# agent-charon/MinGraph-UNet

Hardware: AMD Instinct MI355X
Metric: segmented Mpix/sec, full MinGraph-UNet forward (U-Net + patch-graph GAT), 512x512 batch (higher is better)
Workload: dtype f32

## Files before the change

include/mgunet.h:

```cpp
#ifndef MGUNET_H
#define MGUNET_H

#include <stddef.h>
#include <stdint.h>

#ifdef __cplusplus
extern "C" {
#endif

#define MGU_OK 0
#define MGU_ERR_INVALID -1
#define MGU_ERR_HIP -2
#define MGU_ERR_STATE -3
#define MGU_ERR_NOMEM -4

#define MGU_DTYPE_F32 0
#define MGU_DTYPE_BF16 1

typedef struct mgu_ctx mgu_ctx;

typedef struct {
  const char* name;
  const void* ptr;
  int64_t numel;
// ... 294 lines not shown
                            const float* shift_dev, int act, float* y_dev, int ldy, void* hip_stream);
int mgu_channel_sum_nhwc(mgu_ctx* ctx, const float* x_dev, int ldx, int64_t M, int C, float* out_dev, void* hip_stream);

int mgu_channel_sum_images_nhwc(mgu_ctx* ctx, const float* x_dev, int ldx, int B, int64_t M, int C, float* out_dev, void* hip_stream);

double mgu_unet_flops(mgu_ctx* ctx, int B, int H, int W);
double mgu_unet_mfma_flops(mgu_ctx* ctx, int B, int H, int W);
int mgu_profile_enable(mgu_ctx* ctx, int on);
typedef struct {
  const char* name;
  double ms, flops_alg, flops_mfma;
  int launches, pipe;
} mgu_kernel_stat;
int mgu_profile_read_kernels(mgu_ctx* ctx, mgu_kernel_stat* out, int cap, int* n_out);
int mgu_profile_read(mgu_ctx* ctx, double* conv_ms, int* conv_launches, double* total_ms);

#ifdef __cplusplus
}
#endif
#endif
```

mingraph-unet_amd/csrc/asm/lint_wino_asm.py:

```python
#!/usr/bin/env python3
import re
import sys


def regs(tok):
    tok = tok.strip().lstrip("-").strip("|")
    m = re.match(r"v\[(\d+):(\d+)\]$", tok)
    if m:
        return set(range(int(m.group(1)), int(m.group(2)) + 1))
    m = re.match(r"v(\d+)$", tok)
    return {int(m.group(1))} if m else set()


def parse(line):
    line = line.split(";")[0].strip()
    if not line or line.endswith(":") or line.startswith("."):
        return None
    parts = line.split(None, 1)
    op = parts[0]
    args = []
    if len(parts) > 1:
        a = re.split(r",\s*", parts[1])
        args = [x.split()[0] if x.split() else x for x in a]
    return op, args, line
# ... 50 lines not shown

def loop_bodies(lines):
    lab = {}
    for i, ln in enumerate(lines):
        m = re.match(r"^(\.\w+):", ln)
        if m:
            lab[m.group(1)] = i
    bodies = []
    for i, ln in enumerate(lines):
        m = re.match(r"\s*s_cbranch_scc1\s+(\.\w+)", ln)
        if m and m.group(1) in lab and lab[m.group(1)] < i:
            bodies.append((m.group(1), lines[lab[m.group(1)]:i]))
    return bodies


def replay(stream, errors, where, prime=()):
    vm, lg = [], []
    valu_age = {}
    mfma_age = {}
    prev = None
    m0_fresh = False
    held = {}
    writes = {}

    def age(n):
        for d in (valu_age, mfma_age):
            for r in list(d):
                d[r] += n
                if d[r] > 40:
                    del d[r]

# ... 44 lines not shown
                    errors.append(f"{where}: `{text}` reads v{r} {valu_age[r]} wait state(s) after a VALU write (2 required)")
        else:
            for r in touched if kind in ("valu", "lds_store", "lds_store_addtid", "vm_store", "readlane") else src:
                if r in src and mfma_age.get(r, 99) < 18:
                    errors.append(f"{where}: `{text}` reads MFMA result v{r} after {mfma_age[r]} wait states (18 required)")
        if op.endswith("_dpp"):
            for r in src:
                if valu_age.get(r, 99) < 2:
                    errors.append(f"{where}: `{text}` (DPP) reads v{r} {valu_age[r]} wait state(s) after a VALU write (2 required)")
        if kind == "valu" and prev and prev[0] in ("lds_store", "vm_store") and len(prev[1]) >= 4 and (dst & prev[1]):
            errors.append(f"{where}: `{text}` overwrites store data of the previous instruction `{prev[2]}`")
        if kind == "lds_store_addtid" and m0_fresh:
            errors.append(f"{where}: `{text}` directly behind the write of M0")
        if kind == "readlane" and any(valu_age.get(r, 99) < 1 for r in src):
            errors.append(f"{where}: `{text}` directly behind the VALU write of its source")
        if op in ("v_add_f32_e32", "v_sub_f32_e32"):
            hs = [held.get(r) for a in args[1:3] for r in sorted(regs(a))]
            if len(hs) == 2 and any(h and h[0] == "sum" for h in hs):
                if hs[0] and hs[1] and hs[0] != hs[1]:
                    o = hs[1] if hs[0][0] == "sum" else hs[0]
                    why = f"holds what `{o[1]}` wrote" if o[0] == "other" else \
                          "holds an LDS read, not an inner sum" if o[0] == "lds" else "holds an inner sum of another read base"
                    errors.append(f"{where}: `{text}` combines an inner sum with a register that {why}")
        age(1)
        if kind == "valu":
            for r in dst:
                valu_age[r] = 0
                mfma_age.pop(r, None)
        if kind == "mfma":
            for r in dst:
                mfma_age[r] = 0
# ... 14 lines not shown
        if kind == "vm_load":
            vm.append((dst, text))
        elif kind == "vm_store":
            vm.append((set(), text))
        elif kind == "lds_load":
            lg.append((dst, text))
        elif kind in ("lds_store", "lds_store_addtid"):
            lg.append((set(), text))
        m0_fresh = op == "s_mov_b32" and args and args[0] == "m0"
        data = set()
        if kind in ("lds_store", "vm_store"):
            data = regs(args[1]) if kind == "lds_store" else regs(args[0])
        prev = (kind, data, text)


def check(text):
    errors = []
    ks = kernels(text)
    for name, lines in ks.items():
        replay(lines, errors, f"{name} (straight line)")
        for lab, body in loop_bodies(lines):
            replay(body * 3, errors, f"{name} loop {lab}")
    return errors, len(ks)


if __name__ == "__main__":
    errs, n = check(open(sys.argv[1]).read())
    for e in errs[:40]:
        print(e)
    print(f"{n} kernels, {len(errs)} finding(s)")
    sys.exit(1 if errs else 0)
```

mingraph-unet_amd/csrc/common.h:

```cpp
#pragma once
#include <hip/hip_runtime.h>
#include <stdint.h>

#include "device.h"

namespace mgu {

inline int grid_for(int64_t work, int threads, int cap) {
  int64_t b = (work + threads - 1) / threads;
  if (b < 1) b = 1;
  if (b > cap) b = cap;
  return (int)b;
}
inline bool aligned16(const void* p) { return ((uintptr_t)p & 15) == 0; }

struct Tuning {
  bool first_mfma = true;
  bool use_wino = true;
  int wino_prec = 1;
  bool convt_frag = true;
  bool wino_cp = true;
  int wino_ppb_cap = 32;
  bool wgrad_halo = true;
  bool wino_wgrad = true;
  bool convt_dgrad_x3 = true;
  bool wgrad_x3 = true;
  bool wgrad_thin = true;
  bool wino_dgrad = true;
  bool gat_fused = true;
  bool head_fused = true;
  bool wino_asm = true;
  int fwd_groups = 2;
  int lovasz_passes = 4;
};
const Tuning& default_tuning();
hipError_t ensure_dyn_lds(const void* func, size_t bytes, bool (&done)[64]);

struct IgemmDesc {
  const Tuning* tn;
  const float* in;
  const float* w;
  const float* wu;
  const float* scale;
  const float* shift;
  float* out;
  int M;
// ... 28 lines not shown
};
inline size_t wino_head_psum_bytes(int B, int H, int W) { return (size_t)B * (H / 16) * (W / 16) * 8 * 32 * sizeof(float); }

inline const Tuning& tun(const IgemmDesc& d) { return d.tn ? *d.tn : default_tuning(); }
enum class ConvKernel {
  None,
  WinoAsmWide, WinoAsmCp1r2, WinoAsmCp1r4,
  WinoAsmCp1r2Head,
  WinoCp2, WinoCp1, WinoCp2Stats, WinoCp1Stats,
  WinoCp1Head,
  WinoF32Wide, WinoF32Narrow,
  WinoX3Wide, WinoX3Narrow,
  HaloF32, HaloBf16Np8, HaloBf16Np4,
  TilesF32, TilesBf16,
  ConvtX3, ConvtBf16f, ConvtX3Dgrad,
};
ConvKernel pick_conv(const IgemmDesc& d, int dtype, const WinoHead* head = nullptr);
hipError_t launch_conv(const IgemmDesc& d, ConvKernel k, int dtype, hipStream_t s, const WinoHead* head = nullptr);
inline bool conv_fuses_head(ConvKernel k) { return k == ConvKernel::WinoAsmCp1r2Head || k == ConvKernel::WinoCp1Head; }
inline hipError_t launch_igemm_f32(const IgemmDesc& d, hipStream_t s) { return launch_conv(d, pick_conv(d, 0), 0, s); }
inline hipError_t launch_igemm_bf16(const IgemmDesc& d, hipStream_t s) { return launch_conv(d, pick_conv(d, 1), 1, s); }
const char* conv_kernel_name(ConvKernel k, const IgemmDesc& d);
const char* conv_dgrad_name(ConvKernel k, const IgemmDesc& d);
struct ConvCost {
  double mfma;
  int pipe;
};
ConvCost conv_cost(ConvKernel k, const IgemmDesc& d);
inline bool conv_is_wino(ConvKernel k) { return k >= ConvKernel::WinoAsmWide && k <= ConvKernel::WinoX3Narrow; }
inline bool conv_fuses_pool(ConvKernel k) {
  return conv_is_wino(k) || (k >= ConvKernel::HaloF32 && k <= ConvKernel::HaloBf16Np4);
}
inline bool conv_reads_panel(ConvKernel k) {
  return !conv_is_wino(k) && k != ConvKernel::ConvtX3 && k != ConvKernel::ConvtBf16f && k != ConvKernel::ConvtX3Dgrad;
}
bool wino_layer(const Tuning& t, int KS, int Cp);
bool wino_dgrad_layer(const Tuning& t, int KS, int Cop);
bool convt_x3_layer(const Tuning& t, int Cin, int Cout);
bool convt_x3_dgrad_layer(const Tuning& t, int Cin, int Cout);
bool convt_bf16f_layer(const Tuning& t, int Cin, int Cout);
bool wino_head_layer(const Tuning& t, int dtype, int Cin, int ncls, int patch, int B, int H, int W);
inline bool wino_wide(const IgemmDesc& d) { return d.N > 32; }
struct WinoPlan {
  int tiles_x, tiles_y, total, nblk, ppb, ngroups, per_xcd;
};
WinoPlan wino_plan(const IgemmDesc& d);
int wino_grid_blocks(const IgemmDesc& d);
hipError_t launch_convt_x3(const IgemmDesc& d, hipStream_t s);
hipError_t launch_convt_bf16f(const IgemmDesc& d, hipStream_t s);
hipError_t launch_convt_x3_dgrad(const IgemmDesc& d, hipStream_t s);
bool first_mfma_applicable(int dtype, int Cin, int Cp, int Cout, int ldout, int coff, int64_t H, int64_t W);
hipError_t launch_first_mfma(int dtype, const void* in, const float* wfm, const float* scale, const float* shift, void* out, int B, int H,
                             int W, int ldout, int coff, int relu, hipStream_t s);
hipError_t launch_first_mfma_direct(int dtype, const float* x, int64_t sn, int64_t sc, int64_t sh, int64_t sw, int cin, const float* wfm,
                                    const float* scale, const float* shift, void* out, int B, int H, int W, int ldout, int coff, int relu,
                                    hipStream_t s);
bool first_conv_applicable(int dtype, int Cin, int Cp, int Cout, int ldout, int coff);
hipError_t launch_first_conv(int dtype, const void* in, const float* wf, const float* scale, const float* shift, void* out, int B, int H, int W,
                             int Cin, int Cout, int ldout, int coff, int relu, hipStream_t s);
hipError_t launch_wino_f32(const IgemmDesc& d, ConvKernel k, hipStream_t s, const WinoHead* head = nullptr);
hipError_t launch_patch_sum_combine(const float* psum, float* out, int nodes, hipStream_t s);
hipError_t launch_wino_cp_asm(const IgemmDesc& d, ConvKernel k, hipStream_t s, const WinoHead* head = nullptr);

// ... 136 lines not shown
```

mingraph-unet_amd/csrc/convt_x3.hip:

```cpp
#include <hip/hip_runtime.h>
#include <stdint.h>

#include <algorithm>
#include <type_traits>

#include "common.h"

namespace mgu {


namespace {

template <int MODE, int NI>
__global__ __launch_bounds__(256, 2) void convt2x2_x3_kernel(const float* __restrict__ in, const int ldin, const uint16_t* __restrict__ Wx,
                                                             const float* __restrict__ shift, float* __restrict__ out, const int M,
                                                             const int H, const int W, const int Cin, const int Cout, const int ldout,
                                                             const int coff, const int Hout, const int Wout, const int ntn,
                                                             const int nblocks) {
  constexpr int AP = 40, ABUF = 3 * 128 * AP;
  __shared__ __attribute__((aligned(16))) uint16_t As[2 * ABUF];
  __shared__ int rowoff[128];
  const int chunk = gridDim.x >> 3;
  const int lb = (blockIdx.x & 7) * chunk + (blockIdx.x >> 3);
  if (lb >= nblocks) return;
// ... 169 lines not shown

hipError_t launch_convt_x3_dgrad(const IgemmDesc& d, hipStream_t s) {
  const bool wide = (d.N & 127) == 0;
  const int mtiles = (d.M + 127) / 128, ntn = d.N / (wide ? 128 : 64);
  const int nb = mtiles * ntn;
  const int chunk = (nb + 7) / 8;
  if (wide)
    hipLaunchKernelGGL((convt2x2_x3_kernel<1, 2>), dim3(chunk * 8), dim3(256), 0, s, d.in, d.ldin, reinterpret_cast<const uint16_t*>(d.wu),
                       (const float*)nullptr, d.out, d.M, d.H, d.W, d.Cp, d.N, d.ldout, d.coff, d.Hout, d.Wout, ntn, nb);
  else
    hipLaunchKernelGGL((convt2x2_x3_kernel<1, 1>), dim3(chunk * 8), dim3(256), 0, s, d.in, d.ldin, reinterpret_cast<const uint16_t*>(d.wu),
                       (const float*)nullptr, d.out, d.M, d.H, d.W, d.Cp, d.N, d.ldout, d.coff, d.Hout, d.Wout, ntn, nb);
  return hipGetLastError();
}

hipError_t launch_convt_x3(const IgemmDesc& d, hipStream_t s) {
  const int mtiles = (d.M + 127) / 128, ntn = d.N / 128;
  const int nb = mtiles * ntn;
  const int chunk = (nb + 7) / 8;
  hipLaunchKernelGGL((convt2x2_x3_kernel<0, 2>), dim3(chunk * 8), dim3(256), 0, s, d.in, d.ldin, reinterpret_cast<const uint16_t*>(d.wu), d.shift, d.out,
                     d.M, d.H, d.W, d.Cp, d.ct_cout, d.ldout, d.coff, d.Hout, d.Wout, ntn, nb);
  return hipGetLastError();
}

}
```

mingraph-unet_amd/csrc/ctx.h:

```cpp
#pragma once
#include <stdarg.h>
#include <stdio.h>
#include <stdlib.h>
#include <string.h>

#include <map>
#include <string>
#include <vector>

#include "../../include/mgunet.h"
#include "common.h"

struct Layer {
  std::string prefix;
  std::string conv;
  std::string bn;
  int Cin = 0, Cp = 0, Cout = 0, KS = 3;
  bool convt = false;
  int K = 0, Kp = 0, N = 0, Np = 0;
  float *wp = nullptr, *scale = nullptr, *shift = nullptr;
  bool first = false;
  bool ctb = false;
  bool ctx3 = false;
  bool wino = false;
// ... 82 lines not shown
  hipStream_t comm_stream = nullptr;
  hipEvent_t comm_ev[16] = {};
  int comm_ev_next = 0;
  bool prof = false;
  std::vector<hipEvent_t> ev;
  struct ProfRec {
    const char* name;
    double alg, mfma;
    int pipe;
  };
  std::vector<ProfRec> prec;
  int ev_used = 0;
  hipEvent_t ev_total[2] = {nullptr, nullptr};
  hipStream_t fwd_stream = nullptr;
  hipEvent_t fwd_ev[2] = {nullptr, nullptr};
  int panel_packs = 0;
};

namespace mgud {

inline int rup(int v, int m) { return (v + m - 1) / m * m; }
extern std::string g_create_err;

inline Layer make_layer(int dtype, int Cin, int Cp, int Cout, int KS, bool convt) {
  Layer L;
  L.Cin = Cin, L.Cp = Cp, L.Cout = Cout, L.KS = KS, L.convt = convt;
  L.K = KS * KS * Cp, L.Kp = rup(L.K, dtype == MGU_DTYPE_BF16 ? 64 : 32);
  L.N = convt ? 4 * Cout : Cout, L.Np = rup(L.N, 128);
  return L;
}
// ... 208 lines not shown
```

mingraph-unet_amd/csrc/igemm.hip:

```cpp
#include "common.h"
#include <algorithm>
#include <type_traits>

namespace mgu {


const Tuning& default_tuning() {
  static const Tuning t;
  return t;
}

hipError_t ensure_dyn_lds(const void* func, size_t bytes, bool (&done)[64]) {
  if (bytes <= 65536) return hipSuccess;
  int dev = 0;
  hipError_t e = hipGetDevice(&dev);
  if (e != hipSuccess) return e;
  if (dev < 0 || dev >= 64) return hipFuncSetAttribute(func, hipFuncAttributeMaxDynamicSharedMemorySize, (int)bytes);
  if (done[dev]) return hipSuccess;
  e = hipFuncSetAttribute(func, hipFuncAttributeMaxDynamicSharedMemorySize, (int)bytes);
  if (e == hipSuccess) done[dev] = true;
  return e;
}

template <typename T> struct Elem;
// ... 651 lines not shown

static bool convt_x3_dgrad_applicable(const IgemmDesc& d) {
  return convt_x3_dgrad_layer(tun(d), d.N, d.Cp) && d.KS == 2 && d.wu && d.K == 4 * d.Cp && (d.ldin & 3) == 0 && !d.scale && !d.shift &&
         !d.relu && !d.split_n && !d.pool && (long)d.M * d.ldout < (1l << 31) && (long)d.Hout * d.Wout * d.ldin < (1l << 31);
}

ConvKernel pick_conv(const IgemmDesc& d, int dtype, const WinoHead* head) {
  using K = ConvKernel;
  if (d.M <= 0 || d.N <= 0) return K::None;
  if (dtype == 1) {
    if (d.out_mode == 1) return d.KS != 1 ? K::None : convt_bf16f_applicable(d) ? K::ConvtBf16f : K::TilesBf16;
    const int np = halo_np<__bf16>(d);
    if (np) return np == 8 ? K::HaloBf16Np8 : K::HaloBf16Np4;
    return d.KS == 3 || d.KS == 1 ? K::TilesBf16 : K::None;
  }
  if (d.out_mode == 1) return d.KS != 1 ? K::None : convt_x3_applicable(d) ? K::ConvtX3 : K::TilesF32;
  if (convt_x3_dgrad_applicable(d)) return K::ConvtX3Dgrad;
  if (wino_applicable(d)) {
    const Tuning& t = tun(d);
    const bool wide = wino_wide(d);
    if (!t.wino_prec) return wide ? K::WinoF32Wide : K::WinoF32Narrow;
    if (!t.wino_cp || (long)d.H * d.W * d.ldin * 4 >= 0x7fff0000l) return wide ? K::WinoX3Wide : K::WinoX3Narrow;
    if (d.stat_slots) return wide ? K::WinoCp2Stats : K::WinoCp1Stats;
    if (head && wino_head_applicable(d, *head)) return t.wino_asm ? K::WinoAsmCp1r2Head : K::WinoCp1Head;
    if (wino_asm_applicable(d)) return wide ? K::WinoAsmWide : d.Cp == 32 ? K::WinoAsmCp1r2 : K::WinoAsmCp1r4;
    return wide ? K::WinoCp2 : K::WinoCp1;
  }
  if (halo_np<float>(d) == 8) return K::HaloF32;
  return d.KS >= 1 && d.KS <= 3 ? K::TilesF32 : K::None;
}

// ... 1 lines not shown
  switch (k) {
    case ConvKernel::WinoAsmWide: return "mgu_wino_cp2_gfx950 (asm form of wino3x3_cp_kernel<2>)";
    case ConvKernel::WinoAsmCp1r2: return "mgu_wino_cp1r2_gfx950 (asm form of wino3x3_cp_kernel<1>)";
    case ConvKernel::WinoAsmCp1r4: return "mgu_wino_cp1r4_gfx950 (asm form of wino3x3_cp_kernel<1>)";
    case ConvKernel::WinoAsmCp1r2Head: return "mgu_wino_cp1r2h_gfx950 (asm form of wino3x3_cp_kernel<1, head>: + 1x1 head + patch sums)";
    case ConvKernel::WinoCp1Head: return "wino3x3_cp_kernel<1, head> (+ 1x1 head + patch sums)";
    case ConvKernel::WinoCp2: case ConvKernel::WinoCp2Stats: return "wino3x3_cp_kernel<2>";
    case ConvKernel::WinoCp1: case ConvKernel::WinoCp1Stats: return "wino3x3_cp_kernel<1>";
    case ConvKernel::WinoF32Wide: return "wino3x3_f32_kernel<0,0>";
    case ConvKernel::WinoF32Narrow: return "wino3x3_f32_kernel<1,0>";
    case ConvKernel::WinoX3Wide: return "wino3x3_f32_kernel<0,1>";
    case ConvKernel::WinoX3Narrow: return "wino3x3_f32_kernel<1,1>";
    case ConvKernel::HaloF32: return "conv3x3_halo_kernel<f32>";
    case ConvKernel::HaloBf16Np8: case ConvKernel::HaloBf16Np4: return "conv3x3_halo_kernel<bf16>";
    case ConvKernel::TilesBf16: return d.out_mode == 1 ? "igemm_kernel<bf16> (ConvTranspose)" : "igemm_kernel<bf16>";
    case ConvKernel::ConvtX3: return "convt2x2_x3_kernel";
    case ConvKernel::ConvtBf16f: return "convt2x2_bf16_kernel";
    case ConvKernel::ConvtX3Dgrad: return "convt2x2_x3_kernel<dgrad>";
    case ConvKernel::TilesF32: case ConvKernel::None: break;
  }
  return d.out_mode == 1 ? "igemm_kernel<f32> (ConvTranspose)" : d.KS == 2 ? "igemm_kernel<f32> (ConvTranspose dgrad)" : "igemm_kernel<f32>";
}

const char* conv_dgrad_name(ConvKernel k, const IgemmDesc& d) {
  switch (k) {
    case ConvKernel::WinoAsmWide: case ConvKernel::WinoCp2: case ConvKernel::WinoCp2Stats: return "wino3x3_cp_kernel<2> (dgrad)";
    case ConvKernel::WinoAsmCp1r2: case ConvKernel::WinoAsmCp1r4: case ConvKernel::WinoCp1: case ConvKernel::WinoCp1Stats:
    case ConvKernel::WinoAsmCp1r2Head: case ConvKernel::WinoCp1Head:
      return "wino3x3_cp_kernel<1> (dgrad)";
    case ConvKernel::WinoX3Wide: case ConvKernel::WinoX3Narrow: return "wino3x3_f32_kernel<*,1> (dgrad)";
    case ConvKernel::WinoF32Wide: case ConvKernel::WinoF32Narrow: return "wino3x3_f32_kernel<*,0> (dgrad)";
    case ConvKernel::ConvtX3Dgrad: return "convt2x2_x3_kernel (dgrad)";
    default: return d.KS == 2 ? "igemm_kernel<f32> (ConvTranspose dgrad)" : "igemm/halo (dgrad)";
  }
}

ConvCost conv_cost(ConvKernel k, const IgemmDesc& d) {
  const double direct = 2.0 * d.M * (double)d.K * d.N;
  switch (k) {
    case ConvKernel::WinoF32Wide: case ConvKernel::WinoF32Narrow:
      return {2.0 * (d.M / (d.H * d.W)) * ((d.H + 1) / 2) * ((d.W + 1) / 2) * 16.0 * d.Cp * d.N, 0};
    case ConvKernel::ConvtX3: case ConvKernel::ConvtX3Dgrad: return {6.0 * direct, 1};
    case ConvKernel::HaloBf16Np8: case ConvKernel::HaloBf16Np4: case ConvKernel::TilesBf16: case ConvKernel::ConvtBf16f: return {direct, 1};
    case ConvKernel::HaloF32: case ConvKernel::TilesF32: case ConvKernel::None: return {direct, 0};
    default:
      return {2.0 * (d.M / (d.H * d.W)) * ((d.H + 1) / 2) * ((d.W + 1) / 2) * 16.0 * d.Cp * d.N * 6.0, 1};
  }
}

hipError_t launch_conv(const IgemmDesc& d, ConvKernel k, int dtype, hipStream_t s, const WinoHead* head) {
  if (d.M <= 0 || d.N <= 0) return hipSuccess;
  if (dtype == 1) {
    if ((d.Cp & 7) || (d.ldin & 7) || (d.Kp % 64) || d.K > d.Kp || d.split_n) return hipErrorInvalidValue;
  } else {
    if ((d.Cp & 3) || (d.ldin & 3) || (d.Kp % 32) || d.K > d.Kp) return hipErrorInvalidValue;
  }
  if (conv_fuses_head(k) != (head != nullptr)) return hipErrorInvalidValue;
// ... 5 lines not shown
    case ConvKernel::WinoF32Wide: case ConvKernel::WinoF32Narrow: case ConvKernel::WinoX3Wide: case ConvKernel::WinoX3Narrow:
      return launch_wino_f32(d, k, s);
    case ConvKernel::HaloF32: return launch_halo_tiles<float, 8>(d, s);
    case ConvKernel::HaloBf16Np8: return launch_halo_tiles<__bf16, 8>(d, s);
    case ConvKernel::HaloBf16Np4: return launch_halo_tiles<__bf16, 4>(d, s);
    case ConvKernel::TilesF32:
      if (d.out_mode == 1) return launch_tiles<float, 1, 1>(d, s);
      if (d.KS == 3) return launch_tiles<float, 3, 0>(d, s);
      if (d.KS == 1) return launch_tiles<float, 1, 0>(d, s);
      return launch_tiles<float, 2, 0>(d, s);
    case ConvKernel::TilesBf16:
      if (d.out_mode == 1) return launch_tiles<__bf16, 1, 1>(d, s);
      if (d.KS == 3) return launch_tiles<__bf16, 3, 0>(d, s);
      return launch_tiles<__bf16, 1, 0>(d, s);
    case ConvKernel::ConvtX3: return launch_convt_x3(d, s);
    case ConvKernel::ConvtBf16f: return launch_convt_bf16f(d, s);
    case ConvKernel::ConvtX3Dgrad: return launch_convt_x3_dgrad(d, s);
    case ConvKernel::None: break;
  }
  return hipErrorInvalidValue;
}

}
```

mingraph-unet_amd/csrc/mgunet_api.hip:

```cpp
#include "ctx.h"

#include <algorithm>

using namespace mgu;
using namespace mgud;

namespace mgud {
std::string g_create_err;
}

namespace {

struct WsPlan {
  size_t xin, tmp, tmp_slice, bott, total;
  std::vector<size_t> pooled;
};

int fwd_groups(const mgu_ctx* c, int B) { return c->tn.fwd_groups >= 2 && B >= 2 ? 2 : 1; }
int group_images(const mgu_ctx* c, int B) { return (B + fwd_groups(c, B) - 1) / fwd_groups(c, B); }

WsPlan plan_ws(const mgu_ctx* c, int B, int H, int W) {
  std::vector<int> hs, wsz;
  level_dims(H, W, c->depth, hs, wsz);
  auto out = [&](const Block& b, int l) { return (size_t)B * hs[l] * wsz[l] * c->layers[b.conv2].Cout; };
// ... 62 lines not shown
  Tuning& t = c->tn;
  t.first_mfma = !flag("MGU_NO_FIRST_MFMA");
  t.use_wino = !flag("MGU_NO_WINOGRAD");
  t.wino_prec = num("MGU_WINO_PREC", t.wino_prec) ? 1 : 0;
  t.wino_cp = !flag("MGU_NO_WINO_CP");
  t.convt_frag = !flag("MGU_NO_CONVT_FRAG");
  t.wino_ppb_cap = std::max(1, num("MGU_WINO_PPB_CAP", 32));
  t.wgrad_halo = !flag("MGU_NO_WGRAD_HALO");
  t.wino_wgrad = !flag("MGU_NO_WINO_WGRAD");
  t.wgrad_x3 = !flag("MGU_NO_WGRAD_X3");
  t.convt_dgrad_x3 = !flag("MGU_NO_CONVT_DGRAD_X3");
  t.wgrad_thin = !flag("MGU_NO_THIN_WGRAD");
  t.wino_dgrad = !flag("MGU_NO_WINO_DGRAD");
  t.gat_fused = !flag("MGU_NO_GAT_FUSED");
  t.wino_asm = num("MGU_WINO_ASM", 1) > 0;
  t.head_fused = num("MGU_HEAD_FUSED", 1) > 0;
  t.fwd_groups = num("MGU_FWD_GROUPS", t.fwd_groups) >= 2 ? 2 : 1;
  t.lovasz_passes = num("MGU_LOVASZ_PASSES", t.lovasz_passes) == 3 ? 3 : 4;
  *out = c;
  return MGU_OK;
}

void mgu_destroy(mgu_ctx* c) {
  if (!c) return;
  (void)hipSetDevice(c->device);
  (void)hipDeviceSynchronize();
  (void)mgu_comm_destroy(c);
  if (c->arena) (void)hipFree(c->arena);
  if (c->ws) (void)hipFree(c->ws);
  if (c->gws) (void)hipFree(c->gws);
// ... 285 lines not shown
  if (d.stat_slots || d.pool) k = pick_conv(d, c->dtype, f.head);
  t.head = conv_fuses_head(k);
  const WinoHead* head = t.head ? f.head : nullptr;
  if (took) *took = t;
  if (L.wp_dirty && conv_reads_panel(k)) {
    HIPCHK(c, launch_pack_one(L.convt ? pack_convt_panel(L.w_src, L.wp, c->dtype, L.Cin, L.Cout, L.Kp)
                                      : pack_conv_panel(L.w_src, L.wp, c->dtype, L.Cout, L.Cin, L.Cp, L.KS, L.Kp), s));
    L.wp_dirty = false;
    ++c->panel_packs;
  }
  double alg = L.convt ? 2.0 * d.M * (double)L.Cin * L.Cout * 4.0 : 2.0 * d.M * (double)L.KS * L.KS * L.Cin * L.Cout;
  if (head) alg += 2.0 * d.M * (double)L.Cout * head->ncls;
  const ConvCost cost = conv_cost(k, d);
  ProfScope ps(c, s, conv_kernel_name(k, d), alg, cost.mfma, cost.pipe);
  HIPCHK(c, launch_conv(d, k, c->dtype, s, head));
  return MGU_OK;
}

extern "C" {

int mgu_unet_forward(mgu_ctx* c, const void* x_dev, int B, int H, int W, int64_t xs_n, int64_t xs_c, int64_t xs_h,
                     int64_t xs_w, void* logits_dev, void* const* cat_dev, void* const* feat_dev, int training,
                     void* hip_stream) {
  if (!c) return MGU_ERR_INVALID;
  if (!c->configured || !c->loaded) return fail(c, MGU_ERR_STATE, "configure + load_weights must precede forward");
  if (!x_dev || !logits_dev || !cat_dev || !feat_dev) return fail(c, MGU_ERR_INVALID, "NULL buffer");
  const int depth = c->depth;
  if (B < 1 || H < (1 << depth) || W < (1 << depth))
    return fail(c, MGU_ERR_INVALID, "input %dx%dx%d too small for depth %d", B, H, W, depth);
  if ((int64_t)B * H * W >= (1ll << 31)) return fail(c, MGU_ERR_INVALID, "B*H*W must be < 2^31");
// ... 285 lines not shown
  const size_t panel = (size_t)U.Np * U.Kp + 2 * (size_t)U.Np;
  int rc = ensure(c, &c->gws, &c->gws_bytes, (panel + (x3_shape ? convt_x3_floats(Cin, Cout) : 0)) * sizeof(float));
  if (rc) return rc;
  U.wp = (float*)c->gws;
  U.shift = U.wp + (size_t)U.Np * U.Kp + U.Np;
  U.wu = x3_shape ? U.wp + panel : nullptr;
  HIPCHK(c, hipMemsetAsync(c->gws, 0, panel * sizeof(float), s));
  HIPCHK(c, launch_pack_one(pack_convt_panel((const float*)w_dev, U.wp, 0, Cin, Cout, U.Kp), s));
  IgemmDesc d = layer_desc(c, U, in_dev, Cin, B, H, W, out_dev, ld_out, c_off);
  d.Hout = 2 * H, d.Wout = 2 * W;
  if (bias_dev) {
    HIPCHK(c, launch_pack_one(pack_bias_tile((const float*)bias_dev, U.shift, Cout, 4), s));
    d.shift = U.shift;
  }
  const ConvKernel k = pick_conv(d, 0);
  if (k == ConvKernel::ConvtX3) HIPCHK(c, launch_pack_one(pack_convt_x3((const float*)w_dev, U.wu, Cin, Cout, 0), s));
  ProfScope ps(c, s, conv_kernel_name(k, d));
  HIPCHK(c, launch_conv(d, k, 0, s));
  return MGU_OK;
}

int mgu_maxpool2x2_nhwc(mgu_ctx* c, const void* in_dev, int ld_in, int B, int H, int W, int Cc, void* out_dev,
                        void* hip_stream) {
  if (!c) return MGU_ERR_INVALID;
  if (!in_dev || !out_dev || B < 1 || H < 2 || W < 2 || Cc < 4 || (Cc & 3) || ld_in < Cc || (ld_in & 3))
    return fail(c, MGU_ERR_INVALID, "bad maxpool args (C and ld_in must be multiples of 4, H,W >= 2)");
  HIPCHK(c, hipSetDevice(c->device));
  HIPCHK(c, launch_maxpool2(in_dev, ld_in, out_dev, 0, B, H, W, Cc, (hipStream_t)hip_stream));
  return MGU_OK;
}

int mgu_argmax_classes(mgu_ctx* c, const void* logits_dev, int64_t npix, int num_classes, int64_t* pred_dev,
                       void* hip_stream) {
// ... 49 lines not shown
    const mgu_ctx::ProfRec& r = c->prec[i];
    int k = 0;
    while (k < n && strcmp(out[k].name, r.name) != 0) ++k;
    if (k == n) {
      if (n == cap) continue;
      out[n].name = r.name, out[n].ms = 0, out[n].flops_alg = 0, out[n].flops_mfma = 0, out[n].launches = 0, out[n].pipe = r.pipe;
      ++n;
    }
    out[k].ms += ms, out[k].flops_alg += r.alg, out[k].flops_mfma += r.mfma, out[k].launches += 1;
  }
  *n_out = n;
  c->ev_used = 0;
  return MGU_OK;
}

int mgu_profile_read(mgu_ctx* c, double* conv_ms, int* conv_launches, double* total_ms) {
  if (!c) return MGU_ERR_INVALID;
  if (c->ev_used == 0 || !c->ev_total[1]) return fail(c, MGU_ERR_STATE, "no profiled forward to read");
  HIPCHK(c, hipEventSynchronize(c->ev_total[1]));
  double sum = 0;
  for (int i = 0; i < c->ev_used; ++i) {
    float ms = 0;
    HIPCHK(c, hipEventSynchronize(c->ev[2 * i + 1]));
    HIPCHK(c, hipEventElapsedTime(&ms, c->ev[2 * i], c->ev[2 * i + 1]));
    sum += ms;
  }
  float tot = 0;
  HIPCHK(c, hipEventElapsedTime(&tot, c->ev_total[0], c->ev_total[1]));
  if (conv_ms) *conv_ms = sum;
  if (conv_launches) *conv_launches = c->ev_used;
// ... 6 lines not shown
```

Baseline: 823.8.

## Add hand-scheduled gfx950 assembly kernel for fp32 ConvTranspose x3 path

After: 836.0 (median of 6 runs). 1.01x the previous value.

```diff
diff --git a/include/mgunet.h b/include/mgunet.h
--- a/include/mgunet.h
+++ b/include/mgunet.h
@@ -332,6 +332,7 @@
 } mgu_kernel_stat;
 int mgu_profile_read_kernels(mgu_ctx* ctx, mgu_kernel_stat* out, int cap, int* n_out);
 int mgu_profile_read(mgu_ctx* ctx, double* conv_ms, int* conv_launches, double* total_ms);
+int64_t mgu_convt_asm_launches(mgu_ctx* ctx);
 
 #ifdef __cplusplus
 }
diff --git a/mingraph-unet_amd/csrc/asm/gen_convt_x3.py b/mingraph-unet_amd/csrc/asm/gen_convt_x3.py
--- /dev/null
+++ b/mingraph-unet_amd/csrc/asm/gen_convt_x3.py
@@ -0,0 +1,337 @@
+#!/usr/bin/env python3
+import argparse
+import os
+import sys
+
+sys.path.insert(0, os.path.dirname(os.path.abspath(__file__)))
+from asmkit import Stream, vr, divmod_magic, desc_base, desc_mask
+
+NAME = "mgu_convt_x3_gfx950"
+
+def ACC(mi, ni): return (mi * 2 + ni) * 16
+def BR(buf, f): return 64 + (buf * 6 + f) * 4
+def PA(ss, mi, q): return 112 + ((ss * 2 + mi) * 3 + q) * 4
+def AREG(st, j): return 160 + (st * 4 + j) * 4
+def PCS(j, q): return 192 + (j * 3 + q) * 2
+TB = 216
+VMASK, VST, VRD, VLANE16 = 220, 221, 222, 223
+VAOFF = [224, 225, 226, 227]
+VSH = [228, 229]
+VTID, VROW, VLR4 = 230, 231, 232
+VT = [233, 234, 235, 236, 237, 238, 239]
+def VOFF(mi, g): return AREG(0, 0) + (mi * 4 + g) * 4
+
+S_IN, S_WX, S_OUT, S_SHIFT = 4, 6, 8, 10
+S_W, S_LDIN, S_LDOUT, S_CIN, S_COUT, S_NK, S_NTN, S_NBLOCKS, S_PERXCD, S_WOUT, S_MGNTN, S_MGW, S_MGCOUT, S_PAD = range(12, 26)
+S_T = [26, 27, 28, 29, 30, 31, 32, 33]
+S_NT, S_MT, S_BM0, S_X0, S_WI, S_WM, S_WN = 34, 35, 36, 37, 38, 39, 40
+S_KK, S_NKK1, S_NK1 = 41, 42, 43
+S_INR, S_BRD, S_OUTR, S_SHR = 44, 48, 52, 56
+S_PERM, S_AK, S_BK, S_BK3 = 60, 61, 62, 63
+S_NC = [64, 65]
+S_S, S_LDOUT4, S_LDIN4 = 66, 67, 68
+S_N04 = [69, 70]
+
+ABUF = 3 * 128 * 80
+ROWTAB = 2 * ABUF
+LDS_BYTES, VGPRS, SGPRS, THREADS, KERNARG = ROWTAB + 512, 240, 72, 256, 88
+PRODUCTS = ((2, 0), (0, 2), (1, 1), (1, 0), (0, 1), (0, 0))
+
+
+class Kernel:
+    def __init__(self, o):
+        self.o, self.E, self.L, self.newlabel = o, o.E, o.L, o.newlabel
+        self.end = f".Lend_{NAME}"
+
+
+def emit(kn, ops):
+    for x in ops:
+        kn.E(x)
+
+
+def b_loads(buf):
+    return [f"buffer_load_dwordx4 {vr(BR(buf, f), 4)}, v{VLANE16}, s[{S_BRD}:{S_BRD + 3}], s{S_BK3 if f >= 3 else S_BK} offen offset:{(f % 3) * 1024}"
+            for f in range(6)]
+
+
+def b_advance():
+    return [f"s_add_u32 s{S_KK}, s{S_KK}, 1", f"s_min_u32 s{S_T[0]}, s{S_KK}, s{S_NKK1}", f"s_mul_i32 s{S_BK}, s{S_T[0]}, 0x3000",
+            f"s_add_u32 s{S_BK3}, s{S_BK}, 0xc00"]
+
+
+def a_loads(st):
+    return [f"buffer_load_dwordx4 {vr(AREG(st, j), 4)}, v{VAOFF[j]}, s[{S_INR}:{S_INR + 3}], s{S_AK} offen" for j in range(4)]
+
+
+def a_offset(ahead):
+    return [f"s_add_u32 s{S_T[1]}, s{S_S}, {ahead}", f"s_min_u32 s{S_T[1]}, s{S_T[1]}, s{S_NK1}", f"s_lshl_b32 s{S_AK}, s{S_T[1]}, 7"]
+
+
+def pa_reads(buf, ss):
+    return [f"ds_read_b128 {vr(PA(ss, mi, q), 4)}, v{VRD} offset:{buf * ABUF + (q * 128 + mi * 32) * 80 + ss * 32}"
+            for mi in range(2) for q in range(3)]
+
+
+def split_ops(st, j, buf):
+    a = AREG(st, j)
+    r = []
+    for q in range(3):
+        for p in range(2):
+            r.append(f"v_perm_b32 v{PCS(j, q) + p}, v{a + 2 * p + 1}, v{a + 2 * p}, s{S_PERM}")
+        r.append(f"ds_write_b64 v{VST}, {vr(PCS(j, q), 2)} offset:{buf * ABUF + (q * 128 + j * 32) * 80}")
+        if q < 2:
+            for e in range(4):
+                r.append(f"v_and_b32_e32 v{TB + e}, v{VMASK}, v{a + e}")
+            for e in range(4):
+                r.append(f"v_sub_f32_e32 v{a + e}, v{a + e}, v{TB + e}")
+    assert len(r) == 25
+    return r
+
+
+def mfmas(ss):
+    r = []
+    for mi in range(2):
+        for ni in range(2):
+            acc = vr(ACC(mi, ni), 16)
+            for (pa, pb) in PRODUCTS:
+                r.append(f"v_mfma_f32_32x32x16_bf16 {acc}, {vr(PA(ss, mi, pa), 4)}, {vr(BR(ss, ni * 3 + pb), 4)}, {acc}")
+    return r
+
+
+SPLIT_GAPS = (3, 20)
+
+
+def emit_half(kn, ss, first, spread):
+    g0, g1 = SPLIT_GAPS
+    per = -(-len(spread) // (g1 - g0 + 1))
+    assert per <= 3
+    spread = list(spread)
+    for g, m in enumerate(mfmas(ss)):
+        kn.E(m)
+        emit(kn, first.get(g, []))
+        if g0 <= g <= g1:
+            emit(kn, spread[:per])
+            del spread[:per]
+    assert not spread
+
+
+def emit_step(kn, p):
+    rd = pa_reads(p, 1)
+    first = {g: [x] for g, x in enumerate(b_loads(1))}
+    first[0] = b_advance() + first[0]
+    for g in range(3):
+        first[g] = first[g] + rd[2 * g:2 * g + 2]
+    kn.E("s_waitcnt vmcnt(4) lgkmcnt(0)")
+    emit_half(kn, 0, first, split_ops(p ^ 1, 2, p ^ 1) + split_ops(p ^ 1, 3, p ^ 1))
+    kn.E("s_waitcnt vmcnt(0) lgkmcnt(0)")
+    kn.E("s_barrier")
+    rd = pa_reads(p ^ 1, 0)
+    first = {g: [x] for g, x in enumerate(b_loads(0))}
+    first[0] = b_advance() + first[0]
+    for g in range(3):
+        first[g] = first[g] + rd[2 * g:2 * g + 2]
+    first[5] = first[5] + a_offset(3)
+    for j, x in enumerate(a_loads(p ^ 1)):
+        first[6 + j] = [x]
+    emit_half(kn, 1, first, split_ops(p, 0, p) + split_ops(p, 1, p))
+
+
+def emit_prologue(kn):
+    E, t = kn.E, S_T
+    E("s_load_dwordx16 s[4:19], s[0:1], 0x0")
+    E("s_load_dwordx4 s[20:23], s[0:1], 0x40")
+    E("s_load_dwordx2 s[24:25], s[0:1], 0x50")
+    E(f"v_mov_b32_e32 v{VTID}, v0")
+    E("s_waitcnt lgkmcnt(0)")
+    E(f"s_and_b32 s{t[0]}, s2, 7")
+    E(f"s_mul_i32 s{t[0]}, s{t[0]}, s{S_PERXCD}")
+    E(f"s_lshr_b32 s{t[1]}, s2, 3")
+    E(f"s_add_u32 s{t[0]}, s{t[0]}, s{t[1]}")
+    E(f"s_cmp_ge_u32 s{t[0]}, s{S_NBLOCKS}")
+    E(f"s_cbranch_scc1 {kn.end}")
+    divmod_magic(kn, t[0], S_NTN, S_MGNTN, S_MT, S_NT, t[2], t[3])
+    E(f"s_lshl_b32 s{S_BM0}, s{S_MT}, 7")
+    divmod_magic(kn, S_BM0, S_W, S_MGW, t[4], S_X0, t[2], t[3])
+    E(f"v_lshrrev_b32_e32 v{VT[0]}, 6, v{VTID}")
+    E("s_nop 3")
+    E(f"v_readfirstlane_b32 s{S_WI}, v{VT[0]}")
+    E("s_nop 3")
+    E(f"s_lshr_b32 s{S_WM}, s{S_WI}, 1")
+    E(f"s_and_b32 s{S_WN}, s{S_WI}, 1")
+    E(f"s_mov_b32 s{S_PERM}, 0x07060302")
+    E(f"s_lshl_b32 s{S_LDIN4}, s{S_LDIN}, 2")
+    E(f"s_lshl_b32 s{S_LDOUT4}, s{S_LDOUT}, 2")
+    E(f"s_sub_u32 s{S_NK1}, s{S_NK}, 1")
+    E(f"s_lshl_b32 s{t[4]}, s{S_NK}, 1")
+    E(f"s_sub_u32 s{S_NKK1}, s{t[4]}, 1")
+    desc_base(kn, S_INR, S_IN, S_BM0, S_LDIN4, t[2], t[3])
+    E(f"s_mul_i32 s{t[2]}, s{S_LDIN}, 0x7f")
+    E(f"s_add_u32 s{t[2]}, s{t[2]}, s{S_CIN}")
+    E(f"s_lshl_b32 s{S_INR + 2}, s{t[2]}, 2")
+    E(f"s_mov_b32 s{S_INR + 3}, 0x00020000")
+    E(f"s_mul_i32 s{t[4]}, s{t[4]}, 0x3000")
+    desc_base(kn, S_BRD, S_WX, S_NT, t[4], t[2], t[3], mask=False)
+    E(f"s_mul_i32 s{t[5]}, s{S_WN}, 0x1800")
+    E(f"s_add_u32 s{S_BRD}, s{S_BRD}, s{t[5]}")
+    E(f"s_addc_u32 s{S_BRD + 1}, s{S_BRD + 1}, 0")
+    desc_mask(kn, S_BRD)
+    E(f"s_sub_u32 s{S_BRD + 2}, s{t[4]}, s{t[5]}")
+    E(f"s_mov_b32 s{S_BRD + 3}, 0x00020000")
+    E(f"v_and_b32_e32 v{VT[0]}, 63, v{VTID}")
+    E(f"v_lshlrev_b32_e32 v{VLANE16}, 4, v{VT[0]}")
+    E(f"v_and_b32_e32 v{VT[1]}, 31, v{VT[0]}")
+    E(f"v_lshrrev_b32_e32 v{VT[2]}, 5, v{VT[0]}")
+    E(f"v_lshlrev_b32_e32 v{VLR4}, 2, v{VT[1]}")
+    E(f"s_lshl_b32 s{t[2]}, s{S_WM}, 6")
+    E(f"v_add_u32_e32 v{VT[3]}, s{t[2]}, v{VT[1]}")
+    E(f"v_mul_u32_u24_e32 v{VT[3]}, 0x50, v{VT[3]}")
+    E(f"v_lshl_add_u32 v{VRD}, v{VT[2]}, 4, v{VT[3]}")
+    E(f"s_lshl_b32 s{t[2]}, s{S_WM}, 8")
+    E(f"v_lshlrev_b32_e32 v{VROW}, 4, v{VT[2]}")
+    E(f"v_add_u32_e32 v{VROW}, s{t[2]}, v{VROW}")
+    E(f"v_lshrrev_b32_e32 v{VT[3]}, 3, v{VTID}")
+    E(f"v_and_b32_e32 v{VT[4]}, 7, v{VTID}")
+    E(f"v_mul_u32_u24_e32 v{VST}, 0x50, v{VT[3]}")
+    E(f"v_lshl_add_u32 v{VST}, v{VT[4]}, 3, v{VST}")
+    for j in range(4):
+        E(f"v_add_u32_e32 v{VT[5]}, {j * 32}, v{VT[3]}")
+        E(f"v_mul_lo_u32 v{VT[5]}, v{VT[5]}, s{S_LDIN4}")
+        E(f"v_lshl_add_u32 v{VAOFF[j]}, v{VT[4]}, 4, v{VT[5]}")
+    E(f"v_mov_b32_e32 v{VMASK}, 0xffff0000")
+    E(f"s_lshl_b32 s{t[4]}, s{S_NT}, 7")
+    E(f"s_lshl_b32 s{t[5]}, s{S_WN}, 6")
+    E(f"s_add_u32 s{t[4]}, s{t[4]}, s{t[5]}")
+    for ni in range(2):
+        if ni:
+            E(f"s_add_u32 s{t[4]}, s{t[4]}, 32")
+        E(f"s_lshl_b32 s{S_N04[ni]}, s{t[4]}, 2")
+        divmod_magic(kn, t[4], S_COUT, S_MGCOUT, t[5], t[6], t[3], t[7])
+        E(f"s_lshr_b32 s{t[3]}, s{t[5]}, 1")
+        E(f"s_mul_i32 s{t[3]}, s{t[3]}, s{S_WOUT}")
+        E(f"s_and_b32 s{t[5]}, s{t[5]}, 1")
+        E(f"s_add_u32 s{t[3]}, s{t[3]}, s{t[5]}")
+        E(f"s_mul_i32 s{t[3]}, s{t[3]}, s{S_LDOUT}")
+        E(f"s_add_u32 s{t[3]}, s{t[3]}, s{t[6]}")
+        E(f"s_lshl_b32 s{S_NC[ni]}, s{t[3]}, 2")
+    lnul = kn.newlabel("noshift")
+    E(f"v_mov_b32_e32 v{VSH[0]}, 0")
+    E(f"v_mov_b32_e32 v{VSH[1]}, 0")
+    E(f"s_cmp_eq_u64 s[{S_SHIFT}:{S_SHIFT + 1}], 0")
+    E(f"s_cbranch_scc1 {lnul}")
+    E(f"s_mov_b32 s{S_SHR}, s{S_SHIFT}")
+    desc_mask(kn, S_SHR, S_SHIFT)
+    E(f"s_lshl_b32 s{S_SHR + 2}, s{S_COUT}, 4")
+    E(f"s_mov_b32 s{S_SHR + 3}, 0x00020000")
+    for ni in range(2):
+        E(f"buffer_load_dword v{VSH[ni]}, v{VLR4}, s[{S_SHR}:{S_SHR + 3}], s{S_N04[ni]} offen")
+    kn.L(lnul)
+    E(f"s_mov_b32 s{S_KK}, 0")
+    E(f"s_mov_b32 s{S_S}, 0")
+    E(f"s_mov_b32 s{S_BK}, 0")
+    E(f"s_mov_b32 s{S_BK3}, 0xc00")
+    E(f"s_mov_b32 s{S_AK}, 0")
+    emit(kn, b_loads(0))
+    emit(kn, a_loads(0))
+    emit(kn, a_offset(1))
+    emit(kn, a_loads(1))
+    E(f"v_and_b32_e32 v{VT[0]}, 0x7f, v{VTID}")
+    E(f"v_add_u32_e32 v{VT[1]}, s{S_X0}, v{VT[0]}")
+    E(f"v_mul_hi_u32 v{VT[2]}, v{VT[1]}, s{S_MGW}")
+    E(f"v_mul_lo_u32 v{VT[2]}, v{VT[2]}, s{S_W}")
+    E(f"v_sub_u32_e32 v{VT[1]}, v{VT[1]}, v{VT[2]}")
+    E(f"v_subrev_u32_e32 v{VT[2]}, s{S_W}, v{VT[1]}")
+    E(f"v_cmp_le_u32_e32 vcc, s{S_W}, v{VT[1]}")
+    E("s_nop 1")
+    E(f"v_cndmask_b32_e32 v{VT[1]}, v{VT[1]}, v{VT[2]}, vcc")
+    E(f"v_lshlrev_b32_e32 v{VT[2]}, 2, v{VT[0]}")
+    E(f"v_lshlrev_b32_e32 v{VT[1]}, 1, v{VT[1]}")
+    E(f"v_sub_u32_e32 v{VT[2]}, v{VT[2]}, v{VT[1]}")
+    E(f"s_lshl_b32 s{t[2]}, s{S_X0}, 1")
+    E(f"v_add_u32_e32 v{VT[2]}, s{t[2]}, v{VT[2]}")
+    E(f"v_mul_lo_u32 v{VT[2]}, v{VT[2]}, s{S_LDOUT4}")
+    E(f"v_lshlrev_b32_e32 v{VT[0]}, 2, v{VT[0]}")
+    E(f"ds_write_b32 v{VT[0]}, v{VT[2]} offset:{ROWTAB}")
+    E(f"s_lshl_b32 s{t[4]}, s{S_BM0}, 2")
+    E(f"s_sub_u32 s{t[4]}, s{t[4]}, s{t[2]}")
+    desc_base(kn, S_OUTR, S_OUT, t[4], S_LDOUT4, t[5], t[6])
+    E(f"s_add_u32 s{t[4]}, s{S_X0}, 0x7f")
+    divmod_magic(kn, t[4], S_W, S_MGW, t[5], t[6], t[3], t[7])
+    E(f"s_lshl_b32 s{t[6]}, s{t[6]}, 1")
+    E(f"s_sub_u32 s{t[6]}, 0x1fc, s{t[6]}")
+    E(f"s_add_u32 s{t[6]}, s{t[6]}, s{t[2]}")
+    E(f"s_add_u32 s{t[6]}, s{t[6]}, s{S_WOUT}")
+    E(f"s_add_u32 s{t[6]}, s{t[6]}, 1")
+    E(f"s_mul_i32 s{t[6]}, s{t[6]}, s{S_LDOUT4}")
+    E(f"s_lshl_b32 s{t[5]}, s{S_COUT}, 2")
+    E(f"s_add_u32 s{S_OUTR + 2}, s{t[6]}, s{t[5]}")
+    E(f"s_mov_b32 s{S_OUTR + 3}, 0x00020000")
+    for r in range(64):
+        E(f"v_mov_b32_e32 v{r}, 0")
+    E("s_waitcnt vmcnt(4)")
+    for j in range(4):
+        emit(kn, split_ops(0, j, 0))
+    E("s_waitcnt vmcnt(0)")
+    for j in range(2):
+        emit(kn, split_ops(1, j, 1))
+    emit(kn, a_offset(2))
+    emit(kn, a_loads(0))
+    E("s_waitcnt lgkmcnt(0)")
+    E("s_barrier")
+    emit(kn, pa_reads(0, 0))
+
+
+def emit_epilogue(kn):
+    E = kn.E
+    E("s_waitcnt vmcnt(0) lgkmcnt(0)")
+    for mi in range(2):
+        for g in range(4):
+            E(f"ds_read_b128 {vr(VOFF(mi, g), 4)}, v{VROW} offset:{ROWTAB + (mi * 32 + 8 * g) * 4}")
+    E("s_waitcnt lgkmcnt(0)")
+    for i in range(32):
+        E(f"v_add_u32_e32 v{VOFF(0, 0) + i}, v{VLR4}, v{VOFF(0, 0) + i}")
+    tiles = [(0, 0), (0, 1), (1, 0), (1, 1)]
+    def add(mi, ni, r): return f"v_add_f32_e32 v{ACC(mi, ni) + r}, v{ACC(mi, ni) + r}, v{VSH[ni]}"
+    def store(mi, ni, r):
+        return f"buffer_store_dword v{ACC(mi, ni) + r}, v{VOFF(mi, r >> 2) + (r & 3)}, s[{S_OUTR}:{S_OUTR + 3}], s{S_NC[ni]} offen"
+    for r in range(16):
+        E(add(*tiles[0], r))
+    for k, tl in enumerate(tiles):
+        for r in range(16):
+            E(store(*tl, r))
+            if k + 1 < len(tiles):
+                E(add(*tiles[k + 1], r))
+
+
+def generate():
+    o = Stream()
+    kn = Kernel(o)
+    o.begin_kernel(NAME)
+    emit_prologue(kn)
+    loop, epi = kn.newlabel("step"), kn.newlabel("store")
+    kn.L(loop)
+    emit_step(kn, 0)
+    kn.E(f"s_add_u32 s{S_S}, s{S_S}, 1")
+    kn.E(f"s_cmp_ge_u32 s{S_S}, s{S_NK}")
+    kn.E(f"s_cbranch_scc1 {epi}")
+    emit_step(kn, 1)
+    kn.E(f"s_add_u32 s{S_S}, s{S_S}, 1")
+    kn.E(f"s_cmp_lt_u32 s{S_S}, s{S_NK}")
+    kn.E(f"s_cbranch_scc1 {loop}")
+    kn.L(epi)
+    emit_epilogue(kn)
+    kn.L(kn.end)
+    kn.E("s_endpgm")
+    o.end_kernel(NAME, LDS_BYTES, VGPRS, SGPRS, KERNARG, THREADS)
+    return o.text()
+
+
+def main():
+    ap = argparse.ArgumentParser(description="gfx950 assembly of the fp32 ConvTranspose forward kernel")
+    ap.add_argument("out", metavar="OUT.s")
+    args = ap.parse_args()
+    with open(args.out, "w") as f:
+        f.write(generate())
+
+
+if __name__ == "__main__":
+    main()
diff --git a/mingraph-unet_amd/csrc/asm/lint_wino_asm.py b/mingraph-unet_amd/csrc/asm/lint_wino_asm.py
--- a/mingraph-unet_amd/csrc/asm/lint_wino_asm.py
+++ b/mingraph-unet_amd/csrc/asm/lint_wino_asm.py
@@ -88,7 +88,7 @@
     return bodies
 
 
-def replay(stream, errors, where, prime=()):
+def replay(stream, errors, where, prime=(), shared_sum=True):
     vm, lg = [], []
     valu_age = {}
     mfma_age = {}
@@ -163,7 +163,7 @@
             errors.append(f"{where}: `{text}` directly behind the write of M0")
         if kind == "readlane" and any(valu_age.get(r, 99) < 1 for r in src):
             errors.append(f"{where}: `{text}` directly behind the VALU write of its source")
-        if op in ("v_add_f32_e32", "v_sub_f32_e32"):
+        if shared_sum and op in ("v_add_f32_e32", "v_sub_f32_e32"):
             hs = [held.get(r) for a in args[1:3] for r in sorted(regs(a))]
             if len(hs) == 2 and any(h and h[0] == "sum" for h in hs):
                 if hs[0] and hs[1] and hs[0] != hs[1]:
@@ -208,18 +208,18 @@
         prev = (kind, data, text)
 
 
-def check(text):
+def check(text, shared_sum=True):
     errors = []
     ks = kernels(text)
     for name, lines in ks.items():
-        replay(lines, errors, f"{name} (straight line)")
+        replay(lines, errors, f"{name} (straight line)", shared_sum=shared_sum)
         for lab, body in loop_bodies(lines):
-            replay(body * 3, errors, f"{name} loop {lab}")
+            replay(body * 3, errors, f"{name} loop {lab}", shared_sum=shared_sum)
     return errors, len(ks)
 
 
 if __name__ == "__main__":
-    errs, n = check(open(sys.argv[1]).read())
+    errs, n = check(open(sys.argv[-1]).read(), shared_sum="--no-shared-sum" not in sys.argv[1:-1])
     for e in errs[:40]:
         print(e)
     print(f"{n} kernels, {len(errs)} finding(s)")
diff --git a/mingraph-unet_amd/csrc/common.h b/mingraph-unet_amd/csrc/common.h
--- a/mingraph-unet_amd/csrc/common.h
+++ b/mingraph-unet_amd/csrc/common.h
@@ -30,6 +30,7 @@
   bool gat_fused = true;
   bool head_fused = true;
   bool wino_asm = true;
+  bool convt_asm = true;
   int fwd_groups = 2;
   int lovasz_passes = 4;
 };
@@ -88,6 +89,7 @@
   HaloF32, HaloBf16Np8, HaloBf16Np4,
   TilesF32, TilesBf16,
   ConvtX3, ConvtBf16f, ConvtX3Dgrad,
+  ConvtX3Asm,
 };
 ConvKernel pick_conv(const IgemmDesc& d, int dtype, const WinoHead* head = nullptr);
 hipError_t launch_conv(const IgemmDesc& d, ConvKernel k, int dtype, hipStream_t s, const WinoHead* head = nullptr);
@@ -106,7 +108,11 @@
   return conv_is_wino(k) || (k >= ConvKernel::HaloF32 && k <= ConvKernel::HaloBf16Np4);
 }
 inline bool conv_reads_panel(ConvKernel k) {
-  return !conv_is_wino(k) && k != ConvKernel::ConvtX3 && k != ConvKernel::ConvtBf16f && k != ConvKernel::ConvtX3Dgrad;
+  return !conv_is_wino(k) && k != ConvKernel::ConvtX3 && k != ConvKernel::ConvtX3Asm && k != ConvKernel::ConvtBf16f &&
+         k != ConvKernel::ConvtX3Dgrad;
+}
+inline bool conv_reads_convt_x3(ConvKernel k) {
+  return k == ConvKernel::ConvtX3 || k == ConvKernel::ConvtX3Asm;
 }
 bool wino_layer(const Tuning& t, int KS, int Cp);
 bool wino_dgrad_layer(const Tuning& t, int KS, int Cop);
@@ -121,6 +127,8 @@
 WinoPlan wino_plan(const IgemmDesc& d);
 int wino_grid_blocks(const IgemmDesc& d);
 hipError_t launch_convt_x3(const IgemmDesc& d, hipStream_t s);
+bool convt_x3_asm_shape(const IgemmDesc& d);
+hipError_t launch_convt_x3_asm(const IgemmDesc& d, hipStream_t s);
 hipError_t launch_convt_bf16f(const IgemmDesc& d, hipStream_t s);
 hipError_t launch_convt_x3_dgrad(const IgemmDesc& d, hipStream_t s);
 bool first_mfma_applicable(int dtype, int Cin, int Cp, int Cout, int ldout, int coff, int64_t H, int64_t W);
diff --git a/mingraph-unet_amd/csrc/convt_x3.hip b/mingraph-unet_amd/csrc/convt_x3.hip
--- a/mingraph-unet_amd/csrc/convt_x3.hip
+++ b/mingraph-unet_amd/csrc/convt_x3.hip
@@ -2,9 +2,13 @@
 #include <stdint.h>
 
 #include <algorithm>
+#include <mutex>
 #include <type_traits>
 
 #include "common.h"
+
+extern "C" const unsigned char mgu_convt_x3_hsaco[];
+extern "C" const unsigned mgu_convt_x3_hsaco_len;
 
 namespace mgu {
 
@@ -207,6 +211,62 @@
   return hipGetLastError();
 }
 
+namespace {
+struct ConvtAsmArgs {
+  const float* in;
+  const void* wx;
+  float* out;
+  const float* shift;
+  int W, ldin, ldout, Cin;
+  int Cout, nk, ntn, nblocks;
+  int per_xcd, Wout;
+  unsigned mg_ntn, mg_w;
+  unsigned mg_cout, pad;
+};
+static_assert(sizeof(ConvtAsmArgs) == 88, "kernarg layout of mgu_convt_x3_gfx950");
+unsigned magic(unsigned d) { return d <= 1 ? 0xffffffffu : (unsigned)((1ull << 32) / d); }
+std::mutex g_mu;
+hipModule_t g_mod[64] = {};
+hipFunction_t g_fn[64] = {};
+}
+
+bool convt_x3_asm_shape(const IgemmDesc& d) {
+  if ((d.M & 127) || (d.Cp & 31) || (d.N & 127) || d.Hout != 2 * d.H || d.Wout != 2 * d.W) return false;
+  if ((d.ldin & 3) || (d.ldout & 3) || (d.coff & 3)) return false;
+  if (4l * d.M >= (1l << 31) || 128l * d.ldin * 4 >= (1l << 31) || (9l * 128 + 8l * d.Wout) * d.ldout * 4 >= (1l << 31)) return false;
+  return true;
+}
+
+hipError_t launch_convt_x3_asm(const IgemmDesc& d, hipStream_t s) {
+  int dev = 0;
+  hipError_t e = hipGetDevice(&dev);
+  if (e != hipSuccess) return e;
+  if (dev < 0 || dev >= 64) return hipErrorInvalidDevice;
+  hipFunction_t fn;
+  {
+    std::lock_guard<std::mutex> lk(g_mu);
+    if (!g_mod[dev]) {
+      e = hipModuleLoadData(&g_mod[dev], mgu_convt_x3_hsaco);
+      if (e != hipSuccess) return e;
+    }
+    if (!g_fn[dev]) {
+      e = hipModuleGetFunction(&g_fn[dev], g_mod[dev], "mgu_convt_x3_gfx950");
+      if (e != hipSuccess) return e;
+    }
+    fn = g_fn[dev];
+  }
+  ConvtAsmArgs a;
+  a.in = d.in, a.wx = d.wu, a.out = d.out + d.coff, a.shift = d.shift;
+  a.W = d.W, a.ldin = d.ldin, a.ldout = d.ldout, a.Cin = d.Cp;
+  a.Cout = d.ct_cout, a.nk = d.Cp >> 5, a.ntn = d.N >> 7, a.nblocks = (d.M >> 7) * a.ntn;
+  a.per_xcd = (a.nblocks + 7) / 8, a.Wout = d.Wout;
+  a.mg_ntn = magic((unsigned)a.ntn), a.mg_w = magic((unsigned)d.W);
+  a.mg_cout = magic((unsigned)d.ct_cout), a.pad = 0;
+  size_t sz = sizeof(a);
+  void* extra[] = {HIP_LAUNCH_PARAM_BUFFER_POINTER, &a, HIP_LAUNCH_PARAM_BUFFER_SIZE, &sz, HIP_LAUNCH_PARAM_END};
+  return hipModuleLaunchKernel(fn, (unsigned)(8 * a.per_xcd), 1, 1, 256, 1, 1, 0, s, nullptr, extra);
+}
+
 hipError_t launch_convt_x3(const IgemmDesc& d, hipStream_t s) {
   const int mtiles = (d.M + 127) / 128, ntn = d.N / 128;
   const int nb = mtiles * ntn;
diff --git a/mingraph-unet_amd/csrc/ctx.h b/mingraph-unet_amd/csrc/ctx.h
--- a/mingraph-unet_amd/csrc/ctx.h
+++ b/mingraph-unet_amd/csrc/ctx.h
@@ -120,6 +120,7 @@
   hipEvent_t ev_total[2] = {nullptr, nullptr};
   hipStream_t fwd_stream = nullptr;
   hipEvent_t fwd_ev[2] = {nullptr, nullptr};
+  int64_t convt_asm_launches = 0;
   int panel_packs = 0;
 };
 
diff --git a/mingraph-unet_amd/csrc/igemm.hip b/mingraph-unet_amd/csrc/igemm.hip
--- a/mingraph-unet_amd/csrc/igemm.hip
+++ b/mingraph-unet_amd/csrc/igemm.hip
@@ -689,7 +689,11 @@
     if (np) return np == 8 ? K::HaloBf16Np8 : K::HaloBf16Np4;
     return d.KS == 3 || d.KS == 1 ? K::TilesBf16 : K::None;
   }
-  if (d.out_mode == 1) return d.KS != 1 ? K::None : convt_x3_applicable(d) ? K::ConvtX3 : K::TilesF32;
+  if (d.out_mode == 1) {
+    if (d.KS != 1) return K::None;
+    if (!convt_x3_applicable(d)) return K::TilesF32;
+    return tun(d).convt_asm && convt_x3_asm_shape(d) ? K::ConvtX3Asm : K::ConvtX3;
+  }
   if (convt_x3_dgrad_applicable(d)) return K::ConvtX3Dgrad;
   if (wino_applicable(d)) {
     const Tuning& t = tun(d);
@@ -721,7 +725,7 @@
     case ConvKernel::HaloF32: return "conv3x3_halo_kernel<f32>";
     case ConvKernel::HaloBf16Np8: case ConvKernel::HaloBf16Np4: return "conv3x3_halo_kernel<bf16>";
     case ConvKernel::TilesBf16: return d.out_mode == 1 ? "igemm_kernel<bf16> (ConvTranspose)" : "igemm_kernel<bf16>";
-    case ConvKernel::ConvtX3: return "convt2x2_x3_kernel";
+    case ConvKernel::ConvtX3: case ConvKernel::ConvtX3Asm: return "convt2x2_x3_kernel";
     case ConvKernel::ConvtBf16f: return "convt2x2_bf16_kernel";
     case ConvKernel::ConvtX3Dgrad: return "convt2x2_x3_kernel<dgrad>";
     case ConvKernel::TilesF32: case ConvKernel::None: break;
@@ -747,7 +751,7 @@
   switch (k) {
     case ConvKernel::WinoF32Wide: case ConvKernel::WinoF32Narrow:
       return {2.0 * (d.M / (d.H * d.W)) * ((d.H + 1) / 2) * ((d.W + 1) / 2) * 16.0 * d.Cp * d.N, 0};
-    case ConvKernel::ConvtX3: case ConvKernel::ConvtX3Dgrad: return {6.0 * direct, 1};
+    case ConvKernel::ConvtX3: case ConvKernel::ConvtX3Asm: case ConvKernel::ConvtX3Dgrad: return {6.0 * direct, 1};
     case ConvKernel::HaloBf16Np8: case ConvKernel::HaloBf16Np4: case ConvKernel::TilesBf16: case ConvKernel::ConvtBf16f: return {direct, 1};
     case ConvKernel::HaloF32: case ConvKernel::TilesF32: case ConvKernel::None: return {direct, 0};
     default:
@@ -783,6 +787,7 @@
       if (d.KS == 3) return launch_tiles<__bf16, 3, 0>(d, s);
       return launch_tiles<__bf16, 1, 0>(d, s);
     case ConvKernel::ConvtX3: return launch_convt_x3(d, s);
+    case ConvKernel::ConvtX3Asm: return launch_convt_x3_asm(d, s);
     case ConvKernel::ConvtBf16f: return launch_convt_bf16f(d, s);
     case ConvKernel::ConvtX3Dgrad: return launch_convt_x3_dgrad(d, s);
     case ConvKernel::None: break;
diff --git a/mingraph-unet_amd/csrc/mgunet_api.hip b/mingraph-unet_amd/csrc/mgunet_api.hip
--- a/mingraph-unet_amd/csrc/mgunet_api.hip
+++ b/mingraph-unet_amd/csrc/mgunet_api.hip
@@ -100,6 +100,7 @@
   t.wino_dgrad = !flag("MGU_NO_WINO_DGRAD");
   t.gat_fused = !flag("MGU_NO_GAT_FUSED");
   t.wino_asm = num("MGU_WINO_ASM", 1) > 0;
+  t.convt_asm = num("MGU_CONVT_ASM", 1) > 0;
   t.head_fused = num("MGU_HEAD_FUSED", 1) > 0;
   t.fwd_groups = num("MGU_FWD_GROUPS", t.fwd_groups) >= 2 ? 2 : 1;
   t.lovasz_passes = num("MGU_LOVASZ_PASSES", t.lovasz_passes) == 3 ? 3 : 4;
@@ -415,6 +416,7 @@
   const ConvCost cost = conv_cost(k, d);
   ProfScope ps(c, s, conv_kernel_name(k, d), alg, cost.mfma, cost.pipe);
   HIPCHK(c, launch_conv(d, k, c->dtype, s, head));
+  c->convt_asm_launches += k == ConvKernel::ConvtX3Asm;
   return MGU_OK;
 }
 
@@ -730,9 +732,10 @@
     d.shift = U.shift;
   }
   const ConvKernel k = pick_conv(d, 0);
-  if (k == ConvKernel::ConvtX3) HIPCHK(c, launch_pack_one(pack_convt_x3((const float*)w_dev, U.wu, Cin, Cout, 0), s));
+  if (conv_reads_convt_x3(k)) HIPCHK(c, launch_pack_one(pack_convt_x3((const float*)w_dev, U.wu, Cin, Cout, 0), s));
   ProfScope ps(c, s, conv_kernel_name(k, d));
   HIPCHK(c, launch_conv(d, k, 0, s));
+  c->convt_asm_launches += k == ConvKernel::ConvtX3Asm;
   return MGU_OK;
 }
 
@@ -812,6 +815,8 @@
   return MGU_OK;
 }
 
+int64_t mgu_convt_asm_launches(mgu_ctx* c) { return c ? c->convt_asm_launches : 0; }
+
 int mgu_profile_read(mgu_ctx* c, double* conv_ms, int* conv_launches, double* total_ms) {
   if (!c) return MGU_ERR_INVALID;
   if (c->ev_used == 0 || !c->ev_total[1]) return fail(c, MGU_ERR_STATE, "no profiled forward to read");
```
